# yqtianust/FeatureNet

Measured on AMD Instinct MI355X. Metric: samples/sec (64^3 voxel, 24-class) train, higher is better.
Workload: dtype bf16; 1 GPU; model=FeatureNet-3D, global_batch=128, per_gpu_batch=128, input=64^3x1 voxels, classes=24, parallelism=dp1, impl=native, optimizer=adam, graph=True

## Files before the change

featurenet_amd/csrc/kernels/bind.cpp:

```cpp
#include <hip/hip_runtime.h>
#include <pybind11/pybind11.h>
#include <pybind11/stl.h>

#include <stdexcept>
#include <string>
#include <vector>

namespace py = pybind11;

extern "C" {
int fn_igemm_fwd(const void*, const void*, const float*, void*, float*, const int*, const int*, long long, int, int,
                 int, int, int, hipStream_t, float*, int);
int fn_igemm_fwd_splits(long long, int, int);
int fn_igemm_fwd_mblocks(long long);
int fn_conv_halo(const void*, const void*, const float*, void*, float*, const int*, const int*, int, int, int*,
                 hipStream_t);
long long fn_conv_halo_lds(const int*, int);
int fn_conv_halo_workers(const int*, int);
int fn_pw_fwd(const void*, const void*, const float*, void*, long long, int, int, int, hipStream_t, const float*,
              const float*, int, const void*, const float*, const float*, float*, int);
int fn_seghead_part_len();
int fn_part_reduce(const float*, float*, long long, int, int, hipStream_t);
int fn_seghead_blocks(long long);
int fn_seghead_loss(const void*, const float*, const float*, const void*, const float*, const void*, void*, float*,
// ... 38 lines not shown
int fn_dw_dgrad(const void*, const float*, void*, const int*, hipStream_t);
int fn_dw_wgrad(const void*, const void*, float*, const int*, int, hipStream_t, float*);
int fn_conv_halo_wgrad(const void*, const void*, float*, float*, const int*, int, int, hipStream_t);
int fn_conv_halo_wgrad_gx(const int*, int);
int fn_s2d_pack(const void*, void*, const int*, int, hipStream_t, int);
int fn_dense_splits(int, int, int);
int fn_ew_binary(const void*, const void*, void*, long long, int, hipStream_t);
int fn_ew_mul_bwd(const void*, const void*, const void*, void*, void*, long long, hipStream_t);
int fn_concat2(void*, void*, void*, long long, int, int, int, hipStream_t);
int fn_pad3(void*, void*, const int*, int, hipStream_t);
int fn_pad_channels(void*, void*, long long, int, int, int, hipStream_t);
int fn_dense_fwd(const void*, const void*, const float*, void*, float*, int, int, int, int, int, int, int, hipStream_t);
int fn_dense_dgrad(const void*, const float*, void*, int, int, int, hipStream_t, const void*, int);
int fn_dense_wgrad(const void*, const void*, float*, float*, int, int, int, float*, int, hipStream_t, const void*, int);
int fn_dense_wgrad_slices(int, int, int);
int fn_s2d_weight_map(const float*, float*, const int*, int, hipStream_t);
int fn_subpixel_wmap(const float*, float*, int, int, int, hipStream_t);
int fn_halo_pack_w(const float*, void*, int, int, int, int, int, int, int, hipStream_t);
int fn_igemm_pack_w(const float*, void*, int, int, int, int, int, int, int, int, int, hipStream_t);
int fn_pack_w_multi(const long long*, int, hipStream_t);
int fn_igemm_wgrad(const void*, const void*, float*, const int*, const int*, long long, int, int, int, int,
                   hipStream_t, int, int, const void*, int, float*, int, float*);
long long fn_igemm_wgrad_part(int, int, int, int, int, int, int);
int fn_colstats(const void*, const void*, const float*, const float*, const float*, const float*, float*, long long,
                int, int, int, int, hipStream_t);
int fn_bn_finalize(const float*, int, int, double, const float*, const float*, float*, float*, float, float, float*,
                   float*, float*, float*, int, hipStream_t);
int fn_bn_apply(const void*, const float*, const float*, void*, long long, int, int, hipStream_t, void*);
int fn_bn_wdot(const float*, const float*, float*, int, int, int, hipStream_t);
int fn_bn_bwd_prep(const float*, int, const float*, int, int, double, const float*, const float*, const float*,
// ... 2 lines not shown
int fn_bn_bwd_apply_k_blocks(long long, int);
int fn_bn_bwd_apply_k(const void*, const void*, const float*, const float*, const float*, const float*, void*,
                      long long, int, float*, int, hipStream_t);
int fn_bn_bwd_apply(const void*, const void*, const float*, const float*, const float*, const float*, const float*,
                    const float*, void*, long long, int, float, int, hipStream_t);
int fn_bn_bwd_apply_s2d(const void*, const void*, const float*, const float*, const float*, const float*,
                        const float*, const float*, void*, int, int, int, int, int, float, int, hipStream_t);
int fn_pool_fwd(const void*, void*, const float*, const float*, const int*, int, int, int, hipStream_t);
int fn_pool_bwd(const void*, const void*, void*, const float*, const float*, const int*, int, int, int, hipStream_t);
int fn_pool_bwd_stats_blocks(const int*);
int fn_colstats_blocks(long long, int, int, int);
int fn_pool_bn_bwd_apply(const void*, const void*, const float*, const float*, const float*, const float*,
                         const float*, const float*, void*, const int*, int, float, hipStream_t);
int fn_pool_bwd_stats(const void*, const void*, void*, const float*, const float*, const int*, int, float*,
                      hipStream_t);
int fn_softmax_xent_blocks(long long, int);
int fn_upsample2x(const void*, void*, int, int, int, int, int, int, hipStream_t);
int fn_softmax_xent_rows(const void*, int, const long long*, float*, void*, int*, long long, int, float, float,
                         hipStream_t);
int fn_adam_flat_dev(float*, const float*, float*, float*, void*, long long, const float*, int*, int, hipStream_t);
int fn_adam_flat(float*, const float*, float*, float*, void*, long long, float, float, float, float, float, float,
                 float, float, int, hipStream_t);
int fn_sgd_flat(float*, const float*, float*, void*, long long, float, float, float, int, float, hipStream_t);
int fn_bias_act(const void*, const float*, void*, long long, int, int, hipStream_t);
int fn_act_bwd(const void*, const void*, void*, long long, int, hipStream_t);
int fn_dropout(const void*, void*, long long, float, unsigned, unsigned, hipStream_t);
int fn_cast_f32_bf16(const float*, void*, long long, hipStream_t);
int fn_scale_unless_one(void*, int, const float*, long long, hipStream_t);
int fn_copy2(void*, const void*, long long, void*, const void*, long long, hipStream_t);
int fn_cu_occupy(int, int, int, void*, hipStream_t);
// ... 317 lines not shown
        "dense_fwd");
  }, py::arg("x"), py::arg("w"), py::arg("bias"), py::arg("out"), py::arg("part"), py::arg("M"), py::arg("N"),
     py::arg("K"), py::arg("S"), py::arg("act"), py::arg("out_fp32"), py::arg("st"),
     py::arg("ext") = std::vector<long long>(), py::arg("wbf16") = 0);
  m.def("dense_dgrad", [](uintptr_t g, uintptr_t w, uintptr_t dx, int M, int N, int K, uintptr_t st,
                          std::vector<long long> ext, uintptr_t ya, int act) {
    fits(ext, 0, (long long)M * N, "dense_dgrad", "g");
    fits(ext, 1, (long long)N * K, "dense_dgrad", "w");
    fits(ext, 2, (long long)M * K, "dense_dgrad", "dx");
    if (ya) fits(ext, 3, (long long)M * N, "dense_dgrad", "ya");
    chk(fn_dense_dgrad(P<const void*>(g), P<const float*>(w), P<void*>(dx), M, N, K, S(st), P<const void*>(ya), act),
        "dense_dgrad");
  }, py::arg("g"), py::arg("w"), py::arg("dx"), py::arg("M"), py::arg("N"), py::arg("K"), py::arg("st"),
     py::arg("ext") = std::vector<long long>(), py::arg("ya") = 0, py::arg("act") = 0);
  m.def("dense_wgrad_slices", &fn_dense_wgrad_slices);
  m.def("dense_wgrad", [](uintptr_t g, uintptr_t x, uintptr_t dw, uintptr_t db, int M, int N, int K, uintptr_t st,
                          std::vector<long long> ext, uintptr_t part, int slices, uintptr_t ya, int act) {
    fits(ext, 0, (long long)M * N, "dense_wgrad", "g");
    fits(ext, 1, (long long)M * K, "dense_wgrad", "x");
    fits(ext, 2, (long long)N * K, "dense_wgrad", "dw");
    if (slices > 1) fits(ext, 3, (long long)slices * ((long long)N * K + N), "dense_wgrad", "part");
    if (ya) fits(ext, 4, (long long)M * N, "dense_wgrad", "ya");
    chk(fn_dense_wgrad(P<const void*>(g), P<const void*>(x), P<float*>(dw), P<float*>(db), M, N, K, P<float*>(part),
                       slices, S(st), P<const void*>(ya), act),
        "dense_wgrad");
  }, py::arg("g"), py::arg("x"), py::arg("dw"), py::arg("db"), py::arg("M"), py::arg("N"), py::arg("K"),
     py::arg("st"), py::arg("ext") = std::vector<long long>(), py::arg("part") = 0, py::arg("slices") = 1,
     py::arg("ya") = 0, py::arg("act") = 0);
  m.def("subpixel_wmap", [](uintptr_t src, uintptr_t dst, int K, int C, int mode, uintptr_t st,
                            std::vector<long long> ext) {
// ... 408 lines not shown
  m.def("pool_bwd", [check_pool](uintptr_t dout, uintptr_t x, uintptr_t dx, uintptr_t scale, uintptr_t shift,
                       std::vector<int> geom, int is_max, int count_pad, int act, uintptr_t st,
                       std::vector<long long> ext) {
    need(geom, 17, "pool_bwd");
    check_pool(geom, ext, "pool_bwd");
    chk(fn_pool_bwd(P<const void*>(dout), P<const void*>(x), P<void*>(dx), P<const float*>(scale),
                    P<const float*>(shift), geom.data(), is_max, count_pad, act, S(st)),
        "pool_bwd");
  }, py::arg("dout"), py::arg("x"), py::arg("dx"), py::arg("scale"), py::arg("shift"), py::arg("geom"),
     py::arg("is_max"), py::arg("count_pad"), py::arg("act"), py::arg("st"), py::arg("ext") = std::vector<long long>());
  m.def("pool_bwd_stats_blocks", [](std::vector<int> geom) {
    need(geom, 17, "pool_bwd_stats_blocks");
    return fn_pool_bwd_stats_blocks(geom.data());
  });
  m.def("pool_bwd_stats", [check_pool](uintptr_t dout, uintptr_t x, uintptr_t dx, uintptr_t scale, uintptr_t shift,
                             std::vector<int> geom, int act, uintptr_t part, uintptr_t st, std::vector<long long> ext) {
    need(geom, 17, "pool_bwd_stats");
    check_pool(geom, ext, "pool_bwd_stats");
    fits(ext, 2, 2LL * fn_pool_bwd_stats_blocks(geom.data()) * geom[4], "pool_bwd_stats", "part");
    chk(fn_pool_bwd_stats(P<const void*>(dout), P<const void*>(x), P<void*>(dx), P<const float*>(scale),
                          P<const float*>(shift), geom.data(), act, P<float*>(part), S(st)),
        "pool_bwd_stats");
  }, py::arg("dout"), py::arg("x"), py::arg("dx"), py::arg("scale"), py::arg("shift"), py::arg("geom"),
     py::arg("act"), py::arg("part"), py::arg("st"), py::arg("ext") = std::vector<long long>());
  m.def("pool_bn_bwd_apply", [check_pool](uintptr_t dout, uintptr_t y, uintptr_t scale, uintptr_t shift,
                                uintptr_t mean, uintptr_t invstd, uintptr_t dbeta, uintptr_t dgamma, uintptr_t dy,
                                std::vector<int> geom, int act, float inv_count, uintptr_t st,
                                std::vector<long long> ext) {
    need(geom, 17, "pool_bn_bwd_apply");
    check_pool(geom, ext, "pool_bn_bwd_apply");
    chk(fn_pool_bn_bwd_apply(P<const void*>(dout), P<const void*>(y), P<const float*>(scale), P<const float*>(shift),
                             P<const float*>(mean), P<const float*>(invstd), P<const float*>(dbeta),
                             P<const float*>(dgamma), P<void*>(dy), geom.data(), act, inv_count, S(st)),
        "pool_bn_bwd_apply");
  }, py::arg("dout"), py::arg("y"), py::arg("scale"), py::arg("shift"), py::arg("mean"), py::arg("invstd"),
     py::arg("dbeta"), py::arg("dgamma"), py::arg("dy"), py::arg("geom"), py::arg("act"), py::arg("inv_count"),
     py::arg("st"), py::arg("ext") = std::vector<long long>());
  m.def("upsample2x", [](uintptr_t x, uintptr_t y, int N, int D, int H, int W, int C, int backward, uintptr_t st) {
    chk(fn_upsample2x(P<const void*>(x), P<void*>(y), N, D, H, W, C, backward, S(st)), "upsample2x");
// ... 62 lines not shown
```

featurenet_amd/csrc/kernels/bn_pool.hip:

```cpp
#include "common.h"

#include <algorithm>
#include <type_traits>

template <int VW>
__device__ __forceinline__ void block_moments_to_part(const float (&s0)[VW], const float (&s1)[VW], bool active, int C,
                                                      float* __restrict__ part) {
  __shared__ float red[256][2 * VW + 1];
  const int tid = threadIdx.x;
  const int cpr = C / VW, rpp = 256 / cpr;
#pragma unroll
  for (int j = 0; j < VW; ++j) { red[tid][j] = active ? s0[j] : 0.f; red[tid][VW + j] = active ? s1[j] : 0.f; }
  __syncthreads();
  for (int c = tid; c < C; c += 256) {
    const int chk = c / VW, j = c % VW;
    float a = 0.f, b = 0.f;
    for (int i = 0; i < rpp; ++i) { a += red[i * cpr + chk][j]; b += red[i * cpr + chk][VW + j]; }
    part[(long long)blockIdx.x * 2 * C + c] = a;
    part[(long long)blockIdx.x * 2 * C + C + c] = b;
  }
}

template <int VW>
__device__ __forceinline__ void bn_bwd_consts(int c0, const float* __restrict__ scale, const float* __restrict__ shift,
// ... 527 lines not shown
      }
    }
    const float div = count_pad ? (float)(g.KD * g.KH * g.KW) : (float)(cnt > 0 ? cnt : 1);
    const long long ob = i * VW;
    if constexpr (VW == 8) {
      Pack8 p;
#pragma unroll
      for (int j = 0; j < 8; ++j) p.e[j] = f2bf(is_max ? accv[j] : accv[j] / div);
      *(uint4*)(out + ob) = p.u;
    } else {
      out[ob] = f2bf(is_max ? accv[0] : accv[0] / div);
    }
  }
}

template <int KD, int ACT = -1>
__global__ __launch_bounds__(256) void pool2_fwd_kernel(const bf16* __restrict__ x, bf16* __restrict__ out,
                                                        const float* __restrict__ scale, const float* __restrict__ shift,
                                                        PoolGeom g, int is_max, int act, int total) {
  const int actc = ACT >= 0 ? ACT : act;
  const int cpr = g.C >> 3;
  const int ch = threadIdx.x % cpr;
  float sc[8], sh[8];
#pragma unroll
  for (int j = 0; j < 8; ++j) {
    sc[j] = scale ? scale[ch * 8 + j] : 1.f;
    sh[j] = scale ? shift[ch * 8 + j] : 0.f;
  }
  const long long rowW = (long long)g.W * g.C, plane = (long long)g.H * rowW;
  auto origin = [&](int ii) -> long long {
    int t = ii / cpr;
    const int ow = t % g.OW; t /= g.OW;
    const int oh = t % g.OH; t /= g.OH;
    const int od = t % g.OD;
// ... 4 lines not shown
#pragma unroll
    for (int kd = 0; kd < KD; ++kd)
#pragma unroll
      for (int kh = 0; kh < 2; ++kh)
#pragma unroll
        for (int kw = 0; kw < 2; ++kw) p[(kd * 2 + kh) * 2 + kw].u = *(const uint4*)(x + b0 + kd * plane + kh * rowW + kw * g.C);
  };
  const int stride = gridDim.x * 256;
  int i = blockIdx.x * 256 + threadIdx.x;
  Pack8 p[KD * 4];
  if (i < total) fetch(origin(i), p);
  while (i < total) {
    const int inx = i + stride;
    Pack8 p2[KD * 4];
    fetch(origin(inx < total ? inx : i), p2);
    Pack8 o;
#pragma unroll
    for (int j = 0; j < 8; ++j) {
      float acc = is_max ? -INFINITY : 0.f;
#pragma unroll
      for (int w = 0; w < KD * 4; ++w) {
        float v = bf2f(p[w].e[j]);
        if (scale) v = act_fwd(v * sc[j] + sh[j], actc);
        acc = is_max ? fmaxf(acc, v) : acc + v;
      }
      o.e[j] = f2bf(is_max ? acc : acc * (1.f / (KD * 4)));
    }
    *(uint4*)(out + (long long)i * 8) = o.u;
#pragma unroll
    for (int w = 0; w < KD * 4; ++w) p[w] = p2[w];
    i = inx;
  }
}

template <int VW>
__global__ __launch_bounds__(256) void pool_bwd_kernel(const bf16* __restrict__ dout, const bf16* __restrict__ x,
                                                       bf16* __restrict__ dx, const float* __restrict__ scale,
                                                       const float* __restrict__ shift, PoolGeom g, int is_max,
                                                       int count_pad, int act) {
  const int cpr = g.C / VW;
  const long long total = (long long)g.N * g.D * g.H * g.W * cpr;
  for (long long i = blockIdx.x * 256LL + threadIdx.x; i < total; i += (long long)gridDim.x * 256) {
    const int ch = (int)(i % cpr);
// ... 220 lines not shown
        }
      }
      const float gv = bf2f(pg.e[j]) * act_bwd_from_out(best, actc);
      s0[j] += gv;
      s1[j] += gv * yarg;
    }
    pg = pg2;
#pragma unroll
    for (int w = 0; w < 8; ++w) py[w] = py2[w];
    i = inx;
  }
  block_moments_to_part<8>(s0, s1, true, g.C, part);
}

template <typename I, int ACT = -1>
__global__ __launch_bounds__(256) void pool_bn_bwd_apply_kernel(
    const bf16* __restrict__ dout, const bf16* __restrict__ y, const float* __restrict__ scale,
    const float* __restrict__ shift, const float* __restrict__ mean, const float* __restrict__ invstd,
    const float* __restrict__ dbeta, const float* __restrict__ dgamma, bf16* __restrict__ dy, PoolGeom g, int act,
    float inv_count) {
  const int actc = ACT >= 0 ? ACT : act;
  const int cpr = g.C / 8;
  const I total = (I)g.N * g.OD * g.OH * g.OW * cpr;
  const int win = g.KD * g.KH * g.KW;
  const int ch = (int)(threadIdx.x % cpr);
  float sc[8], sh[8], k2[8], k3[8];
  bn_bwd_consts<8>(ch * 8, scale, shift, mean, invstd, dbeta, dgamma, inv_count, sc, sh, k2, k3);
  I wofs[8];
  pool_win_offsets<I>(g, win, wofs);
  auto origin = [&](I ii) -> I { return pool_win_origin<I>(g, ii, cpr, ch); };
// ... 221 lines not shown
  });
  FN_CHECK_LAUNCH();
  return 0;
}

static PoolGeom pool_geom(const int* g) {
  PoolGeom p;
  p.N = g[0]; p.D = g[1]; p.H = g[2]; p.W = g[3]; p.C = g[4];
  p.OD = g[5]; p.OH = g[6]; p.OW = g[7];
  p.KD = g[8]; p.KH = g[9]; p.KW = g[10];
  p.sd = g[11]; p.sh = g[12]; p.sw = g[13];
  p.pd = g[14]; p.ph = g[15]; p.pw = g[16];
  return p;
}

extern "C" int fn_pool_fwd(const void* x, void* out, const float* scale, const float* shift, const int* geom17,
                           int is_max, int count_pad, int act, hipStream_t st) {
  PoolGeom g = pool_geom(geom17);
  const long long outs = (long long)g.N * g.OD * g.OH * g.OW;
  const bool win2 = g.KH == 2 && g.KW == 2 && (g.KD == 2 || g.KD == 1) && g.sd == g.KD && g.sh == 2 && g.sw == 2 &&
                    g.pd == 0 && g.ph == 0 && g.pw == 0 && g.D >= g.OD * g.KD && g.H >= g.OH * 2 &&
                    g.W >= g.OW * 2 && chunk_fixed(g.C) && outs * (g.C / 8) + 256LL * 8192 < (1LL << 31);
  if (win2) {
    const int total = (int)(outs * (g.C / 8));
    with_int_of<2, 1>(g.KD, [&](auto K) {
      with_act_rn(scale ? act : ACT_NONE, [&](auto A) {
        static const int res = bn_resident_blocks((const void*)pool2_fwd_kernel<K(), A()>);
        hipLaunchKernelGGL((pool2_fwd_kernel<K(), A()>), dim3(resident_grid((total + 255) / 256, res)), dim3(256), 0,
                           st, (const bf16*)x, (bf16*)out, scale, shift, g, is_max, act, total);
      });
    });
  } else
    with_vw(g.C % 8 == 0, [&](auto VW) {
      hipLaunchKernelGGL(pool_fwd_kernel<VW()>, dim3(ew_blocks(outs * (g.C / VW()))), dim3(256), 0, st, (const bf16*)x,
                         (bf16*)out, scale, shift, g, is_max, count_pad, act);
    });
  FN_CHECK_LAUNCH();
// ... 10 lines not shown
  return g.sd == g.KD && g.sh == g.KH && g.sw == g.KW && g.pd == 0 && g.ph == 0 && g.pw == 0 &&
         g.D == g.OD * g.KD && g.H == g.OH * g.KH && g.W == g.OW * g.KW;
}

static bool pool_bwd_stats_ok(const PoolGeom& g) { return pool_tiled(g) && chunk_fixed(g.C); }

extern "C" int fn_pool_bwd_stats_blocks(const int* geom17) {
  const PoolGeom g = pool_geom(geom17);
  if (!pool_bwd_stats_ok(g)) return 0;
  int res = 0;
  if (g.KD * g.KH * g.KW <= 8) {
    static const int r = bn_resident_blocks((const void*)pool_bn_moments8_kernel<int>);
    res = r;
  }
  return resident_rows(((long long)g.N * g.OD * g.OH * g.OW * (g.C / 8) + 255) / 256, res);
}

extern "C" int fn_pool_bwd_stats(const void* dout, const void* x, void* dx, const float* scale, const float* shift,
                                 const int* geom17, int act, float* part, hipStream_t st) {
  const PoolGeom g = pool_geom(geom17);
  const int nb = fn_pool_bwd_stats_blocks(geom17);
  if (nb <= 0 || !scale || !shift || !part) return -2;
  if (!dx && g.KD * g.KH * g.KW <= 8) {
    with_index(pool_i32(g), [&](auto I) {
      with_act_rn(act, [&](auto A) {
        hipLaunchKernelGGL((pool_bn_moments8_kernel<decltype(I), A()>), dim3(nb), dim3(256), 0, st, (const bf16*)dout,
                           (const bf16*)x, scale, shift, g, act, part);
      });
    });
  } else
// ... 78 lines not shown
```

featurenet_amd/csrc/kernels/dense.hip:

```cpp
#include "common.h"

#define DN_THREADS 256
#define DN_WG_MCH 512

__device__ __forceinline__ bf16x8 dn_cvt8(const float4 a, const float4 b) {
  bf16x8 v;
  v[0] = f2bf(a.x); v[1] = f2bf(a.y); v[2] = f2bf(a.z); v[3] = f2bf(a.w);
  v[4] = f2bf(b.x); v[5] = f2bf(b.y); v[6] = f2bf(b.z); v[7] = f2bf(b.w);
  return v;
}

__device__ inline bf16x8 dn_load8(const bf16* __restrict__ row, int c, int n) {
  bf16x8 v = {};
  if ((n & 7) == 0 && c + 8 <= n) return *(const bf16x8*)(row + c);
  if ((n & 3) == 0) {
    if (c + 4 <= n) {
      const bf16x4 a = *(const bf16x4*)(row + c);
      v[0] = a[0]; v[1] = a[1]; v[2] = a[2]; v[3] = a[3];
    }
    if (c + 8 <= n) {
      const bf16x4 b = *(const bf16x4*)(row + c + 4);
      v[4] = b[0]; v[5] = b[1]; v[6] = b[2]; v[7] = b[3];
    }
    return v;
// ... 335 lines not shown
    float* o = dw + (long long)n * K + kk;
    if (kk + 4 <= K && (K & 3) == 0) {
      *(float4*)o = make_float4(acc[j][0], acc[j][1], acc[j][2], acc[j][3]);
    } else {
      for (int e = 0; e < 4; ++e)
        if (kk + e < K) o[e] = acc[j][e];
    }
  }
  if (db && blockIdx.x == 0 && tid < 64) {
#pragma unroll
    for (int b = 0; b < NB; ++b)
      if (n0 + 64 * b + tid < N) db[n0 + 64 * b + tid] = dbs[b];
  }
}

static int dn_ncw(int M, int N, int K) {
  if (N <= 64 || M <= 128) return 1;
  if (K < 512 && ((N + 127) / 128) * ((M + 127) / 128) < 256) return 1;
  return 2;
}

extern "C" int fn_dense_splits(int M, int N, int K) {
  const int ncw = dn_ncw(M, N, K);
  const int tiles = ((N + 64 * ncw - 1) / (64 * ncw)) * ((M + 127) / 128);
  const int target = M <= 128 ? 256 : 512 / ncw;
  int S = (target + tiles - 1) / tiles;
  const int maxS = K / 256 > 0 ? K / 256 : 1;
  return S < 1 ? 1 : (S > maxS ? maxS : S);
}

// ... 48 lines not shown
  }
  FN_CHECK_LAUNCH();
  return 0;
}

static int dn_lds_attr(const void* fn, size_t lds) {
  if (lds <= 64 * 1024) return 0;
  return (int)hipFuncSetAttribute(fn, hipFuncAttributeMaxDynamicSharedMemorySize, (int)lds);
}

extern "C" int fn_dense_dgrad(const void* g, const float* w, void* dx, int M, int N, int K, hipStream_t st,
                              const void* ya, int act) {
  if (M <= 0 || K <= 0 || N <= 0) return -2;
  const size_t lds = (size_t)64 * (((N + 31) & ~31) + 8) * 2;
  if (lds > 160 * 1024) return -4;
  if (int e = dn_lds_attr((const void*)dense_dgrad_kernel, lds)) return e;
  const int mblk = (M + 63) / 64;
  const int mrep = (K + 63) / 64 >= 512 ? (mblk < 4 ? mblk : 4) : 1;
  hipLaunchKernelGGL(dense_dgrad_kernel, dim3((K + 63) / 64, (mblk + mrep - 1) / mrep), dim3(DN_THREADS), lds, st,
                     (const bf16*)g, w, (bf16*)dx, M, N, K, (const bf16*)ya, act, mrep);
  FN_CHECK_LAUNCH();
  return 0;
}

extern "C" int fn_dense_wgrad_slices(int M, int N, int K) {
  const int tiles = ((K + 63) / 64) * ((N + 63) / 64);
  int S = (256 + tiles - 1) / tiles;
  const int maxS = M / 128 > 1 ? M / 128 : 1;
  return S < 1 ? 1 : (S > maxS ? maxS : S);
}

extern "C" int fn_dense_wgrad(const void* g, const void* x, float* dw, float* db, int M, int N, int K, float* part,
                              int S, hipStream_t st, const void* ya, int act) {
  if (M <= 0 || N <= 0 || K <= 0 || S < 1 || (S > 1 && !part)) return -2;
  int mc = (M + S - 1) / S;
  mc = (mc + 31) & ~31;
  S = (M + mc - 1) / mc;
  const int mch = mc < DN_WG_MCH ? mc : DN_WG_MCH;
  const int nb = 1;
  const size_t lds = (size_t)(64 + 64 * nb) * (mch + 8) * 2;
  if (lds > 160 * 1024) return -4;
  const long long NK = (long long)N * K;
  float* pdw = S > 1 ? part : dw;
  float* pdb = S > 1 ? (db ? part + (long long)S * NK : nullptr) : db;
  if (nb == 2) {
    if (int e = dn_lds_attr((const void*)dense_wgrad_kernel<2>, lds)) return e;
    hipLaunchKernelGGL(dense_wgrad_kernel<2>, dim3((K + 63) / 64, (N + 127) / 128, S), dim3(DN_THREADS), lds, st,
                       (const bf16*)g, (const bf16*)x, pdw, pdb, M, N, K, mc, (const bf16*)ya, act);
  } else {
    if (int e = dn_lds_attr((const void*)dense_wgrad_kernel<1>, lds)) return e;
    hipLaunchKernelGGL(dense_wgrad_kernel<1>, dim3((K + 63) / 64, (N + 63) / 64, S), dim3(DN_THREADS), lds, st,
                       (const bf16*)g, (const bf16*)x, pdw, pdb, M, N, K, mc, (const bf16*)ya, act);
  }
  FN_CHECK_LAUNCH();
  if (S > 1) {
    return fn_part_reduce2(part, dw, NK, db ? part + (long long)S * NK : nullptr, db, db ? (long long)N : 0, S, 0, st);
  }
  return 0;
}
```

featurenet_amd/ops/bn.py:

```python
from __future__ import annotations

import torch

from .. import _native
from ..training.flat import grad_target
from . import bnfuse
from . import reference as ref
from .spec import PoolSpec, act_code


def _stats_slab(y2: torch.Tensor) -> torch.Tensor:
    M, C = y2.shape
    nb = _native.kernels().colstats_blocks(M, C, 0, 0)
    part = torch.empty(nb, 2, C, dtype=torch.float32, device=y2.device)
    _native.kernels().colstats(y2.data_ptr(), 0, 0, 0, 0, 0, part.data_ptr(), M, C, 0, 0, nb, _native.stream(y2))
    return part


def _finalize_fwd(slab, count, gamma, beta, rmean, rvar, momentum, eps, update_running=True):
    C = slab.shape[-1]
    out = torch.empty(4, C, dtype=torch.float32, device=slab.device)
    _native.kernels().bn_finalize(
        slab.data_ptr(), slab.shape[0], C, float(count), _native.ptr(gamma), _native.ptr(beta),
        _native.ptr(rmean) if update_running else 0, _native.ptr(rvar) if update_running else 0,
# ... 108 lines not shown
        if isinstance(part, tuple) and ctx.needs_input_grad[0]:
            dy, dbeta, dgamma = _bwd_identity(dz2, y2, prm, *ctx.params, gslab=part[1], wpart=part[2])
            return (dy.reshape(y.shape), dgamma if ctx.has_gamma else None, dbeta if ctx.has_beta else None,
                    None, None, None, None, None, None, None, None)
        dbeta = dgamma = None
        if ctx.training or ctx.needs_input_grad[1] or ctx.needs_input_grad[2]:
            dbeta, dgamma = _bwd_param_grads(dz2, y2, prm, ctx.act, *ctx.params)
        dy = _bwd_input(dz2, y2, prm, dbeta, dgamma, ctx.act, ctx.training) if ctx.needs_input_grad[0] else None
        return (None if dy is None else dy.reshape(y.shape), dgamma if ctx.has_gamma else None,
                dbeta if ctx.has_beta else None, None, None, None, None, None, None, None, None)


class BatchNormActPoolFn(torch.autograd.Function):

    @staticmethod
    def forward(ctx, y, gamma, beta, slab, rmean, rvar, training, momentum, eps, act, pspec, is_max, count_pad):
        C = y.shape[-1]
        y2 = y.reshape(-1, C)
        if training:
            if slab is None:
                slab = _stats_slab(y2)
            prm = _finalize_fwd(slab, y2.shape[0], gamma, beta, rmean, rvar, momentum, eps)
        else:
            prm = _eval_params(gamma, beta, rmean, rvar, eps, C, y.device)
        p = torch.empty(pspec.out_shape5, dtype=torch.bfloat16, device=y.device)
        _native.kernels().pool_fwd(y.data_ptr(), p.data_ptr(), prm[2].data_ptr(), prm[3].data_ptr(), pspec.geom17(),
                                   int(is_max), int(count_pad), act, _native.stream(y), [y.numel(), p.numel()])
        ctx.save_for_backward(y, prm)
        ctx.act, ctx.training, ctx.pspec, ctx.is_max, ctx.count_pad = act, training, pspec, is_max, count_pad
        ctx.has_gamma, ctx.has_beta = gamma is not None, beta is not None
        ctx.params = (beta, gamma)
        return p

    @staticmethod
    def backward(ctx, dp):
        y, prm = ctx.saved_tensors
        C = y.shape[-1]
        dp = dp.contiguous().to(torch.bfloat16)
        K = _native.kernels()
        geom = ctx.pspec.geom17()
        nb = K.pool_bwd_stats_blocks(geom) if (ctx.is_max and ctx.training and bnfuse.pool_stats_enabled()) else 0
        part = None
        ps = ctx.pspec
        if nb > 0 and bnfuse.pool_apply_enabled() and ps.KD * ps.KH * ps.KW <= 8 and C % 8 == 0:
            part = torch.empty(nb, 2, C, dtype=torch.float32, device=y.device)
            K.pool_bwd_stats(dp.data_ptr(), y.data_ptr(), 0, prm[2].data_ptr(), prm[3].data_ptr(), geom, ctx.act,
                             part.data_ptr(), _native.stream(y), [y.numel(), dp.numel(), part.numel()])
            y2 = y.reshape(-1, C)
            dbeta, dgamma = _bwd_param_grads(None, y2, prm, ctx.act, *ctx.params, part=part)
            dy = None
            if ctx.needs_input_grad[0]:
                dy = torch.empty_like(y)
                K.pool_bn_bwd_apply(dp.data_ptr(), y.data_ptr(), prm[2].data_ptr(), prm[3].data_ptr(),
                                    prm[0].data_ptr(), prm[1].data_ptr(), dbeta.data_ptr(), dgamma.data_ptr(),
                                    dy.data_ptr(), geom, ctx.act, 1.0 / y2.shape[0], _native.stream(y),
                                    [y.numel(), dp.numel()])
            return (dy, dgamma if ctx.has_gamma else None, dbeta if ctx.has_beta else None) + (None,) * 10
        dz = torch.empty_like(y)
        if nb > 0:
            part = torch.empty(nb, 2, C, dtype=torch.float32, device=y.device)
            K.pool_bwd_stats(dp.data_ptr(), y.data_ptr(), dz.data_ptr(), prm[2].data_ptr(), prm[3].data_ptr(), geom,
                             ctx.act, part.data_ptr(), _native.stream(y), [y.numel(), dp.numel(), part.numel()])
        else:
            K.pool_bwd(dp.data_ptr(), y.data_ptr(), dz.data_ptr(), prm[2].data_ptr(), prm[3].data_ptr(), geom,
                       int(ctx.is_max), int(ctx.count_pad), ctx.act, _native.stream(y), [y.numel(), dp.numel()])
        y2, dz2 = y.reshape(-1, C), dz.reshape(-1, C)
        dbeta = dgamma = None
        if ctx.training or ctx.needs_input_grad[1] or ctx.needs_input_grad[2]:
            dbeta, dgamma = _bwd_param_grads(dz2, y2, prm, ctx.act, *ctx.params, part=part)
        dy = _bwd_input(dz2, y2, prm, dbeta, dgamma, ctx.act, ctx.training) if ctx.needs_input_grad[0] else None
        return (None if dy is None else dy.reshape(y.shape), dgamma if ctx.has_gamma else None,
                dbeta if ctx.has_beta else None) + (None,) * 10


def batchnorm_act(y5, gamma, beta, running_mean, running_var, training: bool, momentum: float = 0.1,
                  eps: float = 1e-5, act=None, stats_slab=None):
    if _native.use_native(y5):
        tag = training and torch.is_grad_enabled() and (y5.requires_grad or any(
            p is not None and p.requires_grad for p in (gamma, beta)))
        return BatchNormActFn.apply(y5.to(torch.bfloat16).contiguous(), gamma, beta, stats_slab, running_mean,
                                    running_var, training, momentum, eps, act_code(act), tag)
    return ref.batchnorm_act(y5, gamma, beta, running_mean, running_var, training, momentum, eps, act)


def batchnorm_act_pool(y5, gamma, beta, running_mean, running_var, training: bool, pspec: PoolSpec,
                       kind: str = "max", momentum: float = 0.1, eps: float = 1e-5, act=None, stats_slab=None,
                       count_pad: bool = False):
    if _native.use_native(y5):
        return BatchNormActPoolFn.apply(y5.to(torch.bfloat16).contiguous(), gamma, beta, stats_slab, running_mean,
                                        running_var, training, momentum, eps, act_code(act), pspec, kind == "max",
                                        count_pad)
    z = ref.batchnorm_act(y5, gamma, beta, running_mean, running_var, training, momentum, eps, act)
    return ref.pool(z, pspec, kind, count_pad)


class BatchNormActPointwiseFn(torch.autograd.Function):

    @staticmethod
    def forward(ctx, y, gamma, beta, slab, rmean, rvar, momentum, eps, act, w, b):
        from .conv import pw_fwd

        C = y.shape[-1]
        y2 = y.reshape(-1, C)
        if slab is None:
            slab = _stats_slab(y2)
        prm = _finalize_fwd(slab, y2.shape[0], gamma, beta, rmean, rvar, momentum, eps)
# ... 54 lines not shown
```

featurenet_amd/ops/bnfuse.py:

```python
from __future__ import annotations

import os
import threading
import weakref

import torch

_LOCK = threading.Lock()
_FWD: dict = {}
_BWD: dict = {}


def identity_enabled() -> bool:
    return os.environ.get("FN_BN_IDENTITY", "1") != "0"


def identity_ok(C: int, act: int) -> bool:
    return identity_enabled() and act == 1 and C in (32, 64)


def pool_stats_enabled() -> bool:
    return os.environ.get("FN_POOL_BN_STATS", "1") != "0"


def pool_apply_enabled() -> bool:
    return os.environ.get("FN_POOL_BN_APPLY", "1") != "0"


def _purge(d: dict, limit: int = 256) -> None:
    if len(d) > limit:
        for k in [k for k, v in d.items() if v[0]() is None]:
            d.pop(k, None)


def tag_output(z: torch.Tensor, y: torch.Tensor, prm: torch.Tensor, act: int, mask=None) -> None:
    if mask is None:
        return
    with _LOCK:
        _purge(_FWD)
        _FWD[z.data_ptr()] = (weakref.ref(z), weakref.ref(y), weakref.ref(prm), act,
                              weakref.ref(mask) if mask is not None else None)
# ... 31 lines not shown
```

Baseline: 28750 samples/s.

## Save pool argmax inputs for BN backward and add streaming dense dgrad/wgrad kernels

```diff
diff --git a/featurenet_amd/csrc/kernels/bind.cpp b/featurenet_amd/csrc/kernels/bind.cpp
--- a/featurenet_amd/csrc/kernels/bind.cpp
+++ b/featurenet_amd/csrc/kernels/bind.cpp
@@ -76,6 +76,7 @@
 int fn_dense_dgrad(const void*, const float*, void*, int, int, int, hipStream_t, const void*, int);
 int fn_dense_wgrad(const void*, const void*, float*, float*, int, int, int, float*, int, hipStream_t, const void*, int);
 int fn_dense_wgrad_slices(int, int, int);
+int fn_dense_stream(int, int, int, int, int);
 int fn_s2d_weight_map(const float*, float*, const int*, int, hipStream_t);
 int fn_subpixel_wmap(const float*, float*, int, int, int, hipStream_t);
 int fn_halo_pack_w(const float*, void*, int, int, int, int, int, int, int, hipStream_t);
@@ -108,6 +109,9 @@
                          const float*, const float*, void*, const int*, int, float, hipStream_t);
 int fn_pool_bwd_stats(const void*, const void*, void*, const float*, const float*, const int*, int, float*,
                       hipStream_t);
+int fn_pool_arg_ok(const int*);
+int fn_pool_fwd_arg(const void*, void*, void*, const float*, const float*, const int*, int, hipStream_t);
+int fn_pool_arg_moments(const void*, const void*, const float*, const float*, const int*, int, float*, hipStream_t);
 int fn_softmax_xent_blocks(long long, int);
 int fn_upsample2x(const void*, void*, int, int, int, int, int, int, hipStream_t);
 int fn_softmax_xent_rows(const void*, int, const long long*, float*, void*, int*, long long, int, float, float,
@@ -455,6 +459,8 @@
   }, py::arg("g"), py::arg("w"), py::arg("dx"), py::arg("M"), py::arg("N"), py::arg("K"), py::arg("st"),
      py::arg("ext") = std::vector<long long>(), py::arg("ya") = 0, py::arg("act") = 0);
   m.def("dense_wgrad_slices", &fn_dense_wgrad_slices);
+  m.def("dense_stream", &fn_dense_stream, py::arg("kind"), py::arg("M"), py::arg("N"), py::arg("K"),
+        py::arg("has_ya") = 0);
   m.def("dense_wgrad", [](uintptr_t g, uintptr_t x, uintptr_t dw, uintptr_t db, int M, int N, int K, uintptr_t st,
                           std::vector<long long> ext, uintptr_t part, int slices, uintptr_t ya, int act) {
     fits(ext, 0, (long long)M * N, "dense_wgrad", "g");
@@ -893,15 +899,38 @@
     return fn_pool_bwd_stats_blocks(geom.data());
   });
   m.def("pool_bwd_stats", [check_pool](uintptr_t dout, uintptr_t x, uintptr_t dx, uintptr_t scale, uintptr_t shift,
-                             std::vector<int> geom, int act, uintptr_t part, uintptr_t st, std::vector<long long> ext) {
+                             std::vector<int> geom, int act, uintptr_t part, uintptr_t st, std::vector<long long> ext,
+                             uintptr_t yarg) {
     need(geom, 17, "pool_bwd_stats");
     check_pool(geom, ext, "pool_bwd_stats");
     fits(ext, 2, 2LL * fn_pool_bwd_stats_blocks(geom.data()) * geom[4], "pool_bwd_stats", "part");
+    if (yarg) {
+      if (dx) throw std::invalid_argument("pool_bwd_stats: yarg gives the moments only (dx must be 0)");
+      chk(fn_pool_arg_moments(P<const void*>(dout), P<const void*>(yarg), P<const float*>(scale),
+                              P<const float*>(shift), geom.data(), act, P<float*>(part), S(st)),
+          "pool_bwd_stats (yarg)");
+      return;
+    }
     chk(fn_pool_bwd_stats(P<const void*>(dout), P<const void*>(x), P<void*>(dx), P<const float*>(scale),
                           P<const float*>(shift), geom.data(), act, P<float*>(part), S(st)),
         "pool_bwd_stats");
   }, py::arg("dout"), py::arg("x"), py::arg("dx"), py::arg("scale"), py::arg("shift"), py::arg("geom"),
-     py::arg("act"), py::arg("part"), py::arg("st"), py::arg("ext") = std::vector<long long>());
+     py::arg("act"), py::arg("part"), py::arg("st"), py::arg("ext") = std::vector<long long>(),
+     py::arg("yarg") = (uintptr_t)0);
+  m.def("pool_arg_ok", [](std::vector<int> geom) {
+    need(geom, 17, "pool_arg_ok");
+    return fn_pool_arg_ok(geom.data());
+  });
+  m.def("pool_fwd_arg", [check_pool](uintptr_t x, uintptr_t out, uintptr_t yarg, uintptr_t scale, uintptr_t shift,
+                           std::vector<int> geom, int act, uintptr_t st, std::vector<long long> ext) {
+    need(geom, 17, "pool_fwd_arg");
+    check_pool(geom, ext, "pool_fwd_arg");
+    fits(ext, 2, prod({geom[0], geom[5], geom[6], geom[7], geom[4]}), "pool_fwd_arg", "yarg");
+    chk(fn_pool_fwd_arg(P<const void*>(x), P<void*>(out), P<void*>(yarg), P<const float*>(scale),
+                        P<const float*>(shift), geom.data(), act, S(st)),
+        "pool_fwd_arg");
+  }, py::arg("x"), py::arg("out"), py::arg("yarg"), py::arg("scale"), py::arg("shift"), py::arg("geom"),
+     py::arg("act"), py::arg("st"), py::arg("ext") = std::vector<long long>());
   m.def("pool_bn_bwd_apply", [check_pool](uintptr_t dout, uintptr_t y, uintptr_t scale, uintptr_t shift,
                                 uintptr_t mean, uintptr_t invstd, uintptr_t dbeta, uintptr_t dgamma, uintptr_t dy,
                                 std::vector<int> geom, int act, float inv_count, uintptr_t st,
diff --git a/featurenet_amd/csrc/kernels/bn_pool.hip b/featurenet_amd/csrc/kernels/bn_pool.hip
--- a/featurenet_amd/csrc/kernels/bn_pool.hip
+++ b/featurenet_amd/csrc/kernels/bn_pool.hip
@@ -565,10 +565,11 @@
   }
 }
 
-template <int KD, int ACT = -1>
+template <int KD, int ACT = -1, bool ARG = false>
 __global__ __launch_bounds__(256) void pool2_fwd_kernel(const bf16* __restrict__ x, bf16* __restrict__ out,
                                                         const float* __restrict__ scale, const float* __restrict__ shift,
-                                                        PoolGeom g, int is_max, int act, int total) {
+                                                        PoolGeom g, int is_max, int act, int total,
+                                                        bf16* __restrict__ yarg = nullptr) {
   const int actc = ACT >= 0 ? ACT : act;
   const int cpr = g.C >> 3;
   const int ch = threadIdx.x % cpr;
@@ -603,19 +604,24 @@
     const int inx = i + stride;
     Pack8 p2[KD * 4];
     fetch(origin(inx < total ? inx : i), p2);
-    Pack8 o;
+    Pack8 o, oa;
 #pragma unroll
     for (int j = 0; j < 8; ++j) {
       float acc = is_max ? -INFINITY : 0.f;
+      float best = -INFINITY;
+      oa.e[j] = f2bf(0.f);
 #pragma unroll
       for (int w = 0; w < KD * 4; ++w) {
         float v = bf2f(p[w].e[j]);
         if (scale) v = act_fwd(v * sc[j] + sh[j], actc);
         acc = is_max ? fmaxf(acc, v) : acc + v;
+        if constexpr (ARG)
+          if (v > best) { best = v; oa.e[j] = p[w].e[j]; }
       }
       o.e[j] = f2bf(is_max ? acc : acc * (1.f / (KD * 4)));
     }
     *(uint4*)(out + (long long)i * 8) = o.u;
+    if constexpr (ARG) *(uint4*)(yarg + (long long)i * 8) = oa.u;
 #pragma unroll
     for (int w = 0; w < KD * 4; ++w) p[w] = p2[w];
     i = inx;
@@ -866,6 +872,51 @@
 }
 
 template <typename I, int ACT = -1>
+__global__ __launch_bounds__(256) void pool_arg_moments_kernel(const bf16* __restrict__ dout,
+                                                               const bf16* __restrict__ yarg,
+                                                               const float* __restrict__ scale,
+                                                               const float* __restrict__ shift, PoolGeom g, int act,
+                                                               float* __restrict__ part) {
+  const int actc = ACT >= 0 ? ACT : act;
+  const int cpr = g.C / 8;
+  const I total = (I)g.N * g.OD * g.OH * g.OW * cpr;
+  const int ch = (int)(threadIdx.x % cpr);
+  float sc[8], sh[8], s0[8], s1[8];
+#pragma unroll
+  for (int j = 0; j < 8; ++j) {
+    sc[j] = scale[ch * 8 + j];
+    sh[j] = shift[ch * 8 + j];
+    s0[j] = s1[j] = 0.f;
+  }
+  const I stride = (I)gridDim.x * 256;
+  I i = (I)blockIdx.x * 256 + threadIdx.x;
+  Pack8 pg, pa;
+  if (i < total) {
+    pg.u = *(const uint4*)(dout + i * 8);
+    pa.u = *(const uint4*)(yarg + i * 8);
+  }
+  while (i < total) {
+    const I inx = i + stride;
+    const I in2 = inx < total ? inx : i;
+    Pack8 pg2, pa2;
+    pg2.u = *(const uint4*)(dout + in2 * 8);
+    pa2.u = *(const uint4*)(yarg + in2 * 8);
+#pragma unroll
+    for (int j = 0; j < 8; ++j) {
+      const float ya = bf2f(pa.e[j]);
+      const float best = act_fwd(ya * sc[j] + sh[j], actc);
+      const float gv = bf2f(pg.e[j]) * act_bwd_from_out(best, actc);
+      s0[j] += gv;
+      s1[j] += gv * ya;
+    }
+    pg = pg2;
+    pa = pa2;
+    i = inx;
+  }
+  block_moments_to_part<8>(s0, s1, true, g.C, part);
+}
+
+template <typename I, int ACT = -1>
 __global__ __launch_bounds__(256) void pool_bn_bwd_apply_kernel(
     const bf16* __restrict__ dout, const bf16* __restrict__ y, const float* __restrict__ scale,
     const float* __restrict__ shift, const float* __restrict__ mean, const float* __restrict__ invstd,
@@ -1117,13 +1168,18 @@
   return p;
 }
 
+static bool pool_win2(const PoolGeom& g) {
+  const long long outs = (long long)g.N * g.OD * g.OH * g.OW;
+  return g.KH == 2 && g.KW == 2 && (g.KD == 2 || g.KD == 1) && g.sd == g.KD && g.sh == 2 && g.sw == 2 &&
+         g.pd == 0 && g.ph == 0 && g.pw == 0 && g.D >= g.OD * g.KD && g.H >= g.OH * 2 &&
+         g.W >= g.OW * 2 && chunk_fixed(g.C) && outs * (g.C / 8) + 256LL * 8192 < (1LL << 31);
+}
+
 extern "C" int fn_pool_fwd(const void* x, void* out, const float* scale, const float* shift, const int* geom17,
                            int is_max, int count_pad, int act, hipStream_t st) {
   PoolGeom g = pool_geom(geom17);
   const long long outs = (long long)g.N * g.OD * g.OH * g.OW;
-  const bool win2 = g.KH == 2 && g.KW == 2 && (g.KD == 2 || g.KD == 1) && g.sd == g.KD && g.sh == 2 && g.sw == 2 &&
-                    g.pd == 0 && g.ph == 0 && g.pw == 0 && g.D >= g.OD * g.KD && g.H >= g.OH * 2 &&
-                    g.W >= g.OW * 2 && chunk_fixed(g.C) && outs * (g.C / 8) + 256LL * 8192 < (1LL << 31);
+  const bool win2 = pool_win2(g);
   if (win2) {
     const int total = (int)(outs * (g.C / 8));
     with_int_of<2, 1>(g.KD, [&](auto K) {
@@ -1164,6 +1220,42 @@
     res = r;
   }
   return resident_rows(((long long)g.N * g.OD * g.OH * g.OW * (g.C / 8) + 255) / 256, res);
+}
+
+extern "C" int fn_pool_arg_ok(const int* geom17) {
+  const PoolGeom g = pool_geom(geom17);
+  return pool_win2(g) && pool_bwd_stats_ok(g) ? 1 : 0;
+}
+
+extern "C" int fn_pool_fwd_arg(const void* x, void* out, void* yarg, const float* scale, const float* shift,
+                               const int* geom17, int act, hipStream_t st) {
+  const PoolGeom g = pool_geom(geom17);
+  if (!fn_pool_arg_ok(geom17) || !scale || !shift || !yarg) return -2;
+  const int total = (int)((long long)g.N * g.OD * g.OH * g.OW * (g.C / 8));
+  with_int_of<2, 1>(g.KD, [&](auto K) {
+    with_act_rn(act, [&](auto A) {
+      static const int res = bn_resident_blocks((const void*)pool2_fwd_kernel<K(), A(), true>);
+      hipLaunchKernelGGL((pool2_fwd_kernel<K(), A(), true>), dim3(resident_grid((total + 255) / 256, res)), dim3(256),
+                         0, st, (const bf16*)x, (bf16*)out, scale, shift, g, 1, act, total, (bf16*)yarg);
+    });
+  });
+  FN_CHECK_LAUNCH();
+  return 0;
+}
+
+extern "C" int fn_pool_arg_moments(const void* dout, const void* yarg, const float* scale, const float* shift,
+                                   const int* geom17, int act, float* part, hipStream_t st) {
+  const PoolGeom g = pool_geom(geom17);
+  const int nb = fn_pool_bwd_stats_blocks(geom17);
+  if (nb <= 0 || !fn_pool_arg_ok(geom17) || !scale || !shift || !part) return -2;
+  with_index(pool_i32(g), [&](auto I) {
+    with_act_rn(act, [&](auto A) {
+      hipLaunchKernelGGL((pool_arg_moments_kernel<decltype(I), A()>), dim3(nb), dim3(256), 0, st, (const bf16*)dout,
+                         (const bf16*)yarg, scale, shift, g, act, part);
+    });
+  });
+  FN_CHECK_LAUNCH();
+  return 0;
 }
 
 extern "C" int fn_pool_bwd_stats(const void* dout, const void* x, void* dx, const float* scale, const float* shift,
diff --git a/featurenet_amd/csrc/kernels/dense.hip b/featurenet_amd/csrc/kernels/dense.hip
--- a/featurenet_amd/csrc/kernels/dense.hip
+++ b/featurenet_amd/csrc/kernels/dense.hip
@@ -1,4 +1,7 @@
 #include "common.h"
+
+#include <algorithm>
+#include <cstdlib>
 
 #define DN_THREADS 256
 #define DN_WG_MCH 512
@@ -373,6 +376,205 @@
   }
 }
 
+__device__ __forceinline__ int dn_swz(int c, int row, int mask) { return c ^ ((row >> 3) & mask); }
+
+#define DN_DG_OPITCH 72
+#define DN_WG_OPITCH 68
+
+__global__ __launch_bounds__(DN_THREADS) void dense_dgrad_stream_kernel(const bf16* __restrict__ g,
+                                                                        const float* __restrict__ w,
+                                                                        bf16* __restrict__ dx, int M, int N, int K,
+                                                                        int mrep) {
+  extern __shared__ __attribute__((aligned(16))) unsigned char dn_lds[];
+  const int LDN = N + 8;
+  bf16* wt = reinterpret_cast<bf16*>(dn_lds);
+  bf16* gs = wt + 64 * LDN;
+  const int tid = threadIdx.x, lane = tid & 63, wave = tid >> 6;
+  const int r = lane & 15, gq = lane >> 4;
+  const int kk0 = blockIdx.x * 64;
+  const int mbase = blockIdx.y * mrep * 64;
+  const int items = N * 4, gch = N >> 3, gitems = mrep * 64 * gch;
+  auto wload = [&](int idx, float4 (&v)[2][4]) {
+#pragma unroll
+    for (int u = 0; u < 2; ++u) {
+      const int id = idx + u * DN_THREADS;
+      const int q = id & 15, n = (id >> 4) * 4;
+#pragma unroll
+      for (int i = 0; i < 4; ++i)
+        v[u][i] = id < items ? *(const float4*)(w + (long long)(n + i) * K + kk0 + 4 * q)
+                             : make_float4(0.f, 0.f, 0.f, 0.f);
+    }
+  };
+  auto wstore = [&](int idx, const float4 (&v)[2][4]) {
+#pragma unroll
+    for (int u = 0; u < 2; ++u) {
+      const int id = idx + u * DN_THREADS;
+      if (id >= items) break;
+      const int q = id & 15, ng = id >> 4;
+      bf16x4 a[4];
+#pragma unroll
+      for (int i = 0; i < 4; ++i) {
+        a[0][i] = f2bf(v[u][i].x); a[1][i] = f2bf(v[u][i].y); a[2][i] = f2bf(v[u][i].z); a[3][i] = f2bf(v[u][i].w);
+      }
+#pragma unroll
+      for (int e = 0; e < 4; ++e) {
+        const int row = 4 * q + e;
+        *(bf16x4*)(wt + row * LDN + dn_swz(ng >> 1, row, 7) * 8 + (ng & 1) * 4) = a[e];
+      }
+    }
+  };
+  auto gload = [&](int base, uint4 (&t)[8]) {
+#pragma unroll
+    for (int u = 0; u < 8; ++u) {
+      const int id = base + u * DN_THREADS + tid;
+      const int ml = id / gch, c = id - ml * gch;
+      t[u] = make_uint4(0u, 0u, 0u, 0u);
+      if (id < gitems && mbase + ml < M) t[u] = *(const uint4*)(g + (long long)(mbase + ml) * N + 8 * c);
+    }
+  };
+  auto gstore = [&](int base, const uint4 (&t)[8]) {
+#pragma unroll
+    for (int u = 0; u < 8; ++u) {
+      const int id = base + u * DN_THREADS + tid;
+      const int ml = id / gch, c = id - ml * gch;
+      if (id < gitems) *(uint4*)(gs + ml * LDN + 8 * c) = t[u];
+    }
+  };
+  {
+    float4 v[2][4];
+    uint4 t[8];
+    wload(tid, v);
+    gload(0, t);
+    wstore(tid, v);
+    gstore(0, t);
+    for (int idx = tid + 2 * DN_THREADS; idx < items; idx += 2 * DN_THREADS) { wload(idx, v); wstore(idx, v); }
+    for (int base = 8 * DN_THREADS; base < gitems; base += 8 * DN_THREADS) { gload(base, t); gstore(base, t); }
+  }
+  __syncthreads();
+  const int kkw = wave * 16;
+  for (int mi = 0; mi < mrep; ++mi) {
+    const int m0 = mbase + mi * 64;
+    if (m0 >= M) break;
+    bf16* gr = gs + mi * 64 * LDN;
+    f32x4 acc[4];
+#pragma unroll
+    for (int j = 0; j < 4; ++j) acc[j] = (f32x4){0.f, 0.f, 0.f, 0.f};
+    for (int n0 = 0; n0 < N; n0 += 32) {
+      const bf16x8 fa = *(const bf16x8*)(wt + (kkw + r) * LDN + dn_swz((n0 >> 3) + gq, kkw + r, 7) * 8);
+#pragma unroll
+      for (int j = 0; j < 4; ++j) {
+        const bf16x8 v = *(const bf16x8*)(gr + (j * 16 + r) * LDN + n0 + 8 * gq);
+        acc[j] = __builtin_amdgcn_mfma_f32_16x16x32_bf16(fa, v, acc[j], 0, 0, 0);
+      }
+    }
+    __syncthreads();
+#pragma unroll
+    for (int j = 0; j < 4; ++j) {
+      bf16x4 v;
+      v[0] = f2bf(acc[j][0]); v[1] = f2bf(acc[j][1]); v[2] = f2bf(acc[j][2]); v[3] = f2bf(acc[j][3]);
+      *(bf16x4*)(gr + (j * 16 + r) * DN_DG_OPITCH + kkw + 4 * gq) = v;
+    }
+    __syncthreads();
+#pragma unroll
+    for (int p = 0; p < 2; ++p) {
+      const int ml = p * 32 + (tid >> 3), c = tid & 7;
+      if (m0 + ml < M)
+        *(uint4*)(dx + (long long)(m0 + ml) * K + kk0 + 8 * c) = *(const uint4*)(gr + ml * DN_DG_OPITCH + 8 * c);
+    }
+  }
+}
+
+__global__ __launch_bounds__(DN_THREADS) void dense_wgrad_stream_kernel(const bf16* __restrict__ g,
+                                                                        const bf16* __restrict__ x,
+                                                                        float* __restrict__ dw, float* __restrict__ db,
+                                                                        int M, int N, int K, int mc) {
+  extern __shared__ __attribute__((aligned(16))) unsigned char dn_lds[];
+  const int mz0 = blockIdx.z * mc, mz1 = min(M, mz0 + mc);
+  dw += (long long)blockIdx.z * N * K;
+  if (db) db += (long long)blockIdx.z * N;
+  const int MCH = mc < DN_WG_MCH ? ((mc + 31) & ~31) : DN_WG_MCH;
+  const int LDM = MCH + 8;
+  const int cmask = (MCH & 63) ? 3 : 7;
+  bf16* xt = reinterpret_cast<bf16*>(dn_lds);
+  bf16* gt = xt + 64 * LDM;
+  const int tid = threadIdx.x, lane = tid & 63, wave = tid >> 6;
+  const int r = lane & 15, gq = lane >> 4;
+  const int kk0 = blockIdx.x * 64, n0 = blockIdx.y * 64;
+  const int kkw = wave * 16;
+  f32x4 acc[4];
+#pragma unroll
+  for (int j = 0; j < 4; ++j) acc[j] = (f32x4){0.f, 0.f, 0.f, 0.f};
+  float dbs = 0.f;
+  for (int mb = mz0; mb < mz1; mb += MCH) {
+    const int rows = mz1 - mb < MCH ? mz1 - mb : MCH;
+    const int MP = (rows + 31) & ~31;
+    if (mb > mz0) __syncthreads();
+    for (int idx = tid; idx < MP * 2; idx += DN_THREADS) {
+      const int q = idx & 7, mg = idx >> 3;
+      Pack8 vx[4], vg[4];
+#pragma unroll
+      for (int i = 0; i < 4; ++i) {
+        const int ml = 4 * mg + i;
+        vx[i].u = vg[i].u = make_uint4(0u, 0u, 0u, 0u);
+        if (ml < rows) {
+          vx[i].u = *(const uint4*)(x + (long long)(mb + ml) * K + kk0 + 8 * q);
+          vg[i].u = *(const uint4*)(g + (long long)(mb + ml) * N + n0 + 8 * q);
+        }
+      }
+      const int off = dn_swz(mg >> 1, 8 * q, cmask) * 8 + (mg & 1) * 4;
+#pragma unroll
+      for (int e = 0; e < 8; ++e) {
+        bf16x4 a, b;
+#pragma unroll
+        for (int i = 0; i < 4; ++i) { a[i] = vx[i].e[e]; b[i] = vg[i].e[e]; }
+        *(bf16x4*)(xt + (8 * q + e) * LDM + off) = a;
+        *(bf16x4*)(gt + (8 * q + e) * LDM + off) = b;
+      }
+    }
+    __syncthreads();
+    for (int mm = 0; mm < MP; mm += 32) {
+      const int c = (mm >> 3) + gq;
+      const bf16x8 fa = *(const bf16x8*)(xt + (kkw + r) * LDM + dn_swz(c, kkw + r, cmask) * 8);
+#pragma unroll
+      for (int j = 0; j < 4; ++j) {
+        const bf16x8 fb = *(const bf16x8*)(gt + (j * 16 + r) * LDM + dn_swz(c, j * 16 + r, cmask) * 8);
+        acc[j] = __builtin_amdgcn_mfma_f32_16x16x32_bf16(fa, fb, acc[j], 0, 0, 0);
+      }
+    }
+    if (db && blockIdx.x == 0 && tid < 64)
+      for (int m = 0; m < rows; ++m) dbs += bf2f(gt[tid * LDM + dn_swz(m >> 3, tid, cmask) * 8 + (m & 7)]);
+  }
+  __syncthreads();
+  float* ot = reinterpret_cast<float*>(dn_lds);
+#pragma unroll
+  for (int j = 0; j < 4; ++j) *(f32x4*)(ot + (j * 16 + r) * DN_WG_OPITCH + kkw + 4 * gq) = acc[j];
+  __syncthreads();
+#pragma unroll
+  for (int p = 0; p < 4; ++p) {
+    const int n = p * 16 + (tid >> 4), c = tid & 15;
+    *(float4*)(dw + (long long)(n0 + n) * K + kk0 + 4 * c) = *(const float4*)(ot + n * DN_WG_OPITCH + 4 * c);
+  }
+  if (db && blockIdx.x == 0 && tid < 64) db[n0 + tid] = dbs;
+}
+
+static bool dn_stream_on() {
+  const char* e = getenv("FN_DENSE_STREAM");
+  return !(e && e[0] == '0' && e[1] == 0);
+}
+
+static int dn_dgrad_mrep(int M, int K) {
+  const int mblk = (M + 63) / 64;
+  return (K + 63) / 64 >= 512 ? (mblk < 4 ? mblk : 4) : 1;
+}
+
+static size_t dn_dgrad_stream_lds(int M, int N, int K) { return (size_t)(64 + 64 * dn_dgrad_mrep(M, K)) * (N + 8) * 2; }
+
+extern "C" int fn_dense_stream(int kind, int M, int N, int K, int has_ya) {
+  if (!dn_stream_on() || has_ya || M <= 0 || N <= 0 || K <= 0 || K % 64 || N % 64) return 0;
+  if (kind == 1) return dn_dgrad_stream_lds(M, N, K) <= 160 * 1024 ? 1 : 0;
+  return kind == 2 ? 1 : 0;
+}
+
 static int dn_ncw(int M, int N, int K) {
   if (N <= 64 || M <= 128) return 1;
   if (K < 512 && ((N + 127) / 128) * ((M + 127) / 128) < 256) return 1;
@@ -451,9 +653,17 @@
   if (M <= 0 || K <= 0 || N <= 0) return -2;
   const size_t lds = (size_t)64 * (((N + 31) & ~31) + 8) * 2;
   if (lds > 160 * 1024) return -4;
+  const int mblk = (M + 63) / 64;
+  const int mrep = dn_dgrad_mrep(M, K);
+  if (fn_dense_stream(1, M, N, K, ya != nullptr)) {
+    const size_t slds = dn_dgrad_stream_lds(M, N, K);
+    if (int e = dn_lds_attr((const void*)dense_dgrad_stream_kernel, slds)) return e;
+    hipLaunchKernelGGL(dense_dgrad_stream_kernel, dim3(K / 64, (mblk + mrep - 1) / mrep), dim3(DN_THREADS), slds, st,
+                       (const bf16*)g, w, (bf16*)dx, M, N, K, mrep);
+    FN_CHECK_LAUNCH();
+    return 0;
+  }
   if (int e = dn_lds_attr((const void*)dense_dgrad_kernel, lds)) return e;
-  const int mblk = (M + 63) / 64;
-  const int mrep = (K + 63) / 64 >= 512 ? (mblk < 4 ? mblk : 4) : 1;
   hipLaunchKernelGGL(dense_dgrad_kernel, dim3((K + 63) / 64, (mblk + mrep - 1) / mrep), dim3(DN_THREADS), lds, st,
                      (const bf16*)g, w, (bf16*)dx, M, N, K, (const bf16*)ya, act, mrep);
   FN_CHECK_LAUNCH();
@@ -480,7 +690,12 @@
   const long long NK = (long long)N * K;
   float* pdw = S > 1 ? part : dw;
   float* pdb = S > 1 ? (db ? part + (long long)S * NK : nullptr) : db;
-  if (nb == 2) {
+  if (fn_dense_stream(2, M, N, K, ya != nullptr)) {
+    const size_t slds = std::max(lds, (size_t)64 * DN_WG_OPITCH * 4);
+    if (int e = dn_lds_attr((const void*)dense_wgrad_stream_kernel, slds)) return e;
+    hipLaunchKernelGGL(dense_wgrad_stream_kernel, dim3(K / 64, N / 64, S), dim3(DN_THREADS), slds, st,
+                       (const bf16*)g, (const bf16*)x, pdw, pdb, M, N, K, mc);
+  } else if (nb == 2) {
     if (int e = dn_lds_attr((const void*)dense_wgrad_kernel<2>, lds)) return e;
     hipLaunchKernelGGL(dense_wgrad_kernel<2>, dim3((K + 63) / 64, (N + 127) / 128, S), dim3(DN_THREADS), lds, st,
                        (const bf16*)g, (const bf16*)x, pdw, pdb, M, N, K, mc, (const bf16*)ya, act);
diff --git a/featurenet_amd/ops/bn.py b/featurenet_amd/ops/bn.py
--- a/featurenet_amd/ops/bn.py
+++ b/featurenet_amd/ops/bn.py
@@ -146,7 +146,8 @@
 class BatchNormActPoolFn(torch.autograd.Function):
 
     @staticmethod
-    def forward(ctx, y, gamma, beta, slab, rmean, rvar, training, momentum, eps, act, pspec, is_max, count_pad):
+    def forward(ctx, y, gamma, beta, slab, rmean, rvar, training, momentum, eps, act, pspec, is_max, count_pad,
+                save_arg=False):
         C = y.shape[-1]
         y2 = y.reshape(-1, C)
         if training:
@@ -156,9 +157,17 @@
         else:
             prm = _eval_params(gamma, beta, rmean, rvar, eps, C, y.device)
         p = torch.empty(pspec.out_shape5, dtype=torch.bfloat16, device=y.device)
-        _native.kernels().pool_fwd(y.data_ptr(), p.data_ptr(), prm[2].data_ptr(), prm[3].data_ptr(), pspec.geom17(),
-                                   int(is_max), int(count_pad), act, _native.stream(y), [y.numel(), p.numel()])
-        ctx.save_for_backward(y, prm)
+        yarg = None
+        if save_arg:
+            yarg = torch.empty_like(p)
+            _native.kernels().pool_fwd_arg(y.data_ptr(), p.data_ptr(), yarg.data_ptr(), prm[2].data_ptr(),
+                                           prm[3].data_ptr(), pspec.geom17(), act, _native.stream(y),
+                                           [y.numel(), p.numel(), yarg.numel()])
+        else:
+            _native.kernels().pool_fwd(y.data_ptr(), p.data_ptr(), prm[2].data_ptr(), prm[3].data_ptr(),
+                                       pspec.geom17(), int(is_max), int(count_pad), act, _native.stream(y),
+                                       [y.numel(), p.numel()])
+        ctx.save_for_backward(y, prm, yarg)
         ctx.act, ctx.training, ctx.pspec, ctx.is_max, ctx.count_pad = act, training, pspec, is_max, count_pad
         ctx.has_gamma, ctx.has_beta = gamma is not None, beta is not None
         ctx.params = (beta, gamma)
@@ -166,7 +175,7 @@
 
     @staticmethod
     def backward(ctx, dp):
-        y, prm = ctx.saved_tensors
+        y, prm, yarg = ctx.saved_tensors
         C = y.shape[-1]
         dp = dp.contiguous().to(torch.bfloat16)
         K = _native.kernels()
@@ -177,7 +186,8 @@
         if nb > 0 and bnfuse.pool_apply_enabled() and ps.KD * ps.KH * ps.KW <= 8 and C % 8 == 0:
             part = torch.empty(nb, 2, C, dtype=torch.float32, device=y.device)
             K.pool_bwd_stats(dp.data_ptr(), y.data_ptr(), 0, prm[2].data_ptr(), prm[3].data_ptr(), geom, ctx.act,
-                             part.data_ptr(), _native.stream(y), [y.numel(), dp.numel(), part.numel()])
+                             part.data_ptr(), _native.stream(y), [y.numel(), dp.numel(), part.numel()],
+                             _native.ptr(yarg))
             y2 = y.reshape(-1, C)
             dbeta, dgamma = _bwd_param_grads(None, y2, prm, ctx.act, *ctx.params, part=part)
             dy = None
@@ -187,7 +197,7 @@
                                     prm[0].data_ptr(), prm[1].data_ptr(), dbeta.data_ptr(), dgamma.data_ptr(),
                                     dy.data_ptr(), geom, ctx.act, 1.0 / y2.shape[0], _native.stream(y),
                                     [y.numel(), dp.numel()])
-            return (dy, dgamma if ctx.has_gamma else None, dbeta if ctx.has_beta else None) + (None,) * 10
+            return (dy, dgamma if ctx.has_gamma else None, dbeta if ctx.has_beta else None) + (None,) * 11
         dz = torch.empty_like(y)
         if nb > 0:
             part = torch.empty(nb, 2, C, dtype=torch.float32, device=y.device)
@@ -202,7 +212,7 @@
             dbeta, dgamma = _bwd_param_grads(dz2, y2, prm, ctx.act, *ctx.params, part=part)
         dy = _bwd_input(dz2, y2, prm, dbeta, dgamma, ctx.act, ctx.training) if ctx.needs_input_grad[0] else None
         return (None if dy is None else dy.reshape(y.shape), dgamma if ctx.has_gamma else None,
-                dbeta if ctx.has_beta else None) + (None,) * 10
+                dbeta if ctx.has_beta else None) + (None,) * 11
 
 
 def batchnorm_act(y5, gamma, beta, running_mean, running_var, training: bool, momentum: float = 0.1,
@@ -219,9 +229,13 @@
                        kind: str = "max", momentum: float = 0.1, eps: float = 1e-5, act=None, stats_slab=None,
                        count_pad: bool = False):
     if _native.use_native(y5):
+        save_arg = (training and kind == "max" and torch.is_grad_enabled() and bnfuse.pool_arg_enabled()
+                    and bnfuse.pool_stats_enabled() and bnfuse.pool_apply_enabled()
+                    and (y5.requires_grad or any(p is not None and p.requires_grad for p in (gamma, beta)))
+                    and bool(_native.kernels().pool_arg_ok(pspec.geom17())))
         return BatchNormActPoolFn.apply(y5.to(torch.bfloat16).contiguous(), gamma, beta, stats_slab, running_mean,
                                         running_var, training, momentum, eps, act_code(act), pspec, kind == "max",
-                                        count_pad)
+                                        count_pad, save_arg)
     z = ref.batchnorm_act(y5, gamma, beta, running_mean, running_var, training, momentum, eps, act)
     return ref.pool(z, pspec, kind, count_pad)
 
diff --git a/featurenet_amd/ops/bnfuse.py b/featurenet_amd/ops/bnfuse.py
--- a/featurenet_amd/ops/bnfuse.py
+++ b/featurenet_amd/ops/bnfuse.py
@@ -25,6 +25,10 @@
 
 def pool_apply_enabled() -> bool:
     return os.environ.get("FN_POOL_BN_APPLY", "1") != "0"
+
+
+def pool_arg_enabled() -> bool:
+    return os.environ.get("FN_POOL_ARG", "1") != "0"
 
 
 def _purge(d: dict, limit: int = 256) -> None:
```

After: 29000 samples/s (median of 6 runs). About the same (+0.9%).
